# lisqzqng/Video-based-gait-analysis-for-dementia

Hardware: AMD Instinct MI355X
Metric: frames/sec (224x224, seq=16) (higher is better)
Workload: dtype f32

## Files before the change

include/grnet_hip.h:

```cpp
#ifndef GRNET_HIP_H
#define GRNET_HIP_H

#include <stddef.h>
#include <stdint.h>

#ifdef __cplusplus
extern "C" {
#endif

typedef struct grnet grnet_t;

#define GRNET_OK 0
#define GRNET_EINVAL (-22)
#define GRNET_ENOENT (-2)
#define GRNET_ENOMEM (-12)
#define GRNET_EHIP (-5)
#define GRNET_ESTATE (-1)

#define GRNET_DTYPE_F32 0
#define GRNET_DTYPE_I64 1

int grnet_create(grnet_t** out_handle, int device_id, int dtype, int max_frames);

#define GRNET_PRECISION_F32 0
// ... 7 lines not shown
int grnet_arena_fill(grnet_t* h, uint32_t pattern, void* stream);
int grnet_arena_assign(int n, const int64_t* sizes, int n_pairs, const int32_t* conflict_pairs, int64_t* offsets, int64_t* total);

int grnet_load_tensor(grnet_t* h, const char* state_dict_key, const void* host_ptr, const int64_t* shape, int ndim,
                      int dtype);

int grnet_load_smpl(grnet_t* h, const float* v_template, const float* shapedirs, const float* posedirs,
                    const float* J_regressor, const float* lbs_weights, const int32_t* parents,
                    const float* J_regressor_extra);

int grnet_finalize_weights(grnet_t* h);

typedef struct grnet_outputs {
    float* theta;
    float* verts;
    float* kp_2d;
    float* kp_3d;
    float* rotmat;
    float* point_local_feat;
    float* cam_shape_feats;
    float* pred_rot6d;
    float* features;
    float* part_attn;
    float* smpl_feats;
} grnet_outputs_t;

int grnet_forward(grnet_t* h, const float* frames_dev, int n_frames, const grnet_outputs_t* out, void* stream);

int grnet_gru_forward(grnet_t* h, const float* x_dev, const float* cparams_dev, int b, int T, float* y_dev,
                      float* phase_dev, float* xc_dev, void* stream);

int grnet_tsattn_forward(grnet_t* h, const float* x_dev, const float* xs_dev, int b, int n, float* y_dev, void* stream);

int grnet_tsattn_plan(grnet_t* h, int n, int32_t* plan);

int grnet_temporal_taps(grnet_t* h, float* buf_dev, size_t floats);

int grnet_temporal_tap_layout(grnet_t* h, char* buf, int buf_size);

#define GRNET_OPT_USE_GRAPH 1
#define GRNET_OPT_CONV_TILE 2
#define GRNET_OPT_MULTI_LANE 3
#define GRNET_OPT_WINOGRAD 7
#define GRNET_OPT_BF16_CHAIN 8
#define GRNET_OPT_GRU_MODE 9
#define GRNET_OPT_BF16_MIN_FRAMES 10
int grnet_set_option(grnet_t* h, int option, int value);

int grnet_tune(grnet_t* h, int n_frames, void* stream, int level );
int grnet_get_tuning(grnet_t* h, int n_frames, char* buf, int buf_size);
int grnet_set_tuning(grnet_t* h, int n_frames, const char* text);

int grnet_num_kernel_launches(grnet_t* h);
int grnet_num_conv_launches(grnet_t* h);
double grnet_conv_flops_per_frame(grnet_t* h);
double grnet_conv_executed_flops_per_frame(grnet_t* h);
double grnet_conv_executed_flops_per_frame_n(grnet_t* h, int n_frames);
int grnet_describe_conv(grnet_t* h, int pos, int32_t* info , char* name, int name_size);
double grnet_describe_conv_macs(grnet_t* h, int pos);
int grnet_conv_kernel_info(grnet_t* h, int pos, int n_frames, char* name, int name_size, double* executed_macs_per_frame);
int grnet_time_conv(grnet_t* h, int pos, int n_frames, int reps, void* stream, float* us_out);
int grnet_conv_launch_form(grnet_t* h, int pos, int n_frames, char* buf, int size, int* tuning_index);
int grnet_op_timeline(grnet_t* h, const float* frames_dev, int n_frames, void* stream, char* buf, int buf_size);
int grnet_time_convs(grnet_t* h, int n_frames, void* stream, float* ms_out);

int grnet_op_conv2d(grnet_t* h, const float* in_dev, int n, int cin, int hgt, int wid, const float* w_host,
                    const float* bias_host, int cout, int ks, int stride, int relu, const float* add_dev,
                    float* out_dev, int tile_hint, void* stream);
int grnet_op_conv2d_adds(grnet_t* h, const float* in_dev, int n, int cin, int hgt, int wid, const float* w_host, const float* bias_host, int cout, int ks,
                         int stride, int relu, int n_add, const float* const* adds_dev, const int* add_ctot, const int* add_coff, const int* add_shift,
                         float* out_dev, int tile_hint, void* stream);
int grnet_op_bilinear2x(grnet_t* h, const float* in_dev, int n, int c, int hgt, int wid, float* out_dev, void* stream);
int grnet_op_conv_chain(grnet_t* h, const float* in_dev, int n, int c, int wid, int nconv, const float* w_host, const float* bias_host,
                        float* out_dev, int reps, float* us_out, void* stream);

int grnet_smpl_forward(grnet_t* h, const float* betas_dev, const float* rotmat_dev, const float* cam_dev, int n, float* verts_dev,
                       float* kp3d_dev, float* kp2d_dev, void* stream);

#define GRNET_JOINT_REGRESSOR_MAX_ROWS 64
int grnet_set_joint_regressor(grnet_t* h, const float* J_host, int rows, const int32_t* select, int n_select);
int grnet_joint_regressor_rows(grnet_t* h);
int grnet_regress_joints(grnet_t* h, const float* verts_dev, int n, float* joints_dev, void* stream);

int grnet_head_forward(grnet_t* h, const float* point_local_feat_dev, const float* cam_shape_feats_dev, int n, const grnet_outputs_t* out,
                       void* stream);
typedef struct grnet_gait_outputs {
    float* pred_avg;
    float* pred_phase;
    float* pred_cparam;
    float* point_local_feat;
} grnet_gait_outputs_t;
int grnet_gait_correct(grnet_t* h, const float* point_local_feat_dev, const float* cam_shape_feats_dev, const float* cam_dev, int cam_ld,
                       const float* bbox_dev, const float* cimg_dev, int b, int T, const grnet_outputs_t* out,
                       const grnet_gait_outputs_t* gait, void* stream);

int grnet_op_rot6d_to_rotmat(grnet_t* h, const float* rot6d_dev, int m, float* rotmat_dev, void* stream);
int grnet_op_rotmat_to_aa(grnet_t* h, const float* rotmat_dev, int m, float* aa_dev, void* stream);
int grnet_op_aa_to_rotmat(grnet_t* h, const float* aa_dev, int m, float* rotmat_dev, void* stream);

int grnet_op_one_euro(grnet_t* h, const float* x_dev, int ld, int T, float min_cutoff, float beta, float d_cutoff, float* xhat_dev, void* stream);

#define GRNET_JOINTS_SPIN49   0
#define GRNET_JOINTS_SPIN2    1
#define GRNET_JOINTS_KINECTV2 2
int grnet_smooth_pose(grnet_t* h, const float* pose_dev, int pose_ld, const float* betas_dev, int T, float min_cutoff, float beta, int joints_kind,
                      float* pose_hat_dev, float* verts_dev, float* joints_dev, void* stream);
// ... 39 lines not shown
```

video-based-gait-analysis-for-dementia_amd/_lib.py:

```python
import ctypes as C
import os

_HERE = os.path.dirname(os.path.abspath(__file__))
LIB_PATH = os.environ.get("GRNET_LIB_PATH") or os.path.join(_HERE, "libgrnet_hip.so")

OK, EINVAL, ENOENT, ENOMEM, EHIP, ESTATE = 0, -22, -2, -12, -5, -1
DTYPE_F32, DTYPE_I64 = 0, 1
PRECISION_F32, PRECISION_BF16 = 0, 1
CREATE_COMPACT_ARENA = 1
JOINT_REGRESSOR_MAX_ROWS = 64
JOINTS_SPIN49, JOINTS_SPIN2, JOINTS_KINECTV2 = 0, 1, 2
RASTER_MAX_DIM, RASTER_SLOTS = 4096, 16
OPT_USE_GRAPH, OPT_CONV_TILE, OPT_MULTI_LANE, OPT_WINOGRAD, OPT_BF16_CHAIN, OPT_GRU_MODE, OPT_BF16_MIN_FRAMES = 1, 2, 3, 7, 8, 9, 10


class Outputs(C.Structure):
    _fields_ = [(n, C.c_void_p) for n in (
        "theta", "verts", "kp_2d", "kp_3d", "rotmat", "point_local_feat", "cam_shape_feats", "pred_rot6d",
        "features", "part_attn", "smpl_feats")]


class GaitOutputs(C.Structure):
    _fields_ = [(n, C.c_void_p) for n in ("pred_avg", "pred_phase", "pred_cparam", "point_local_feat")]


EXPORTS = {
    "grnet_create": (C.c_int, [C.POINTER(C.c_void_p), C.c_int, C.c_int, C.c_int]),
    "grnet_create_ex": (C.c_int, [C.POINTER(C.c_void_p), C.c_int, C.c_int, C.c_int, C.c_uint]),
    "grnet_arena_query": (C.c_int, [C.c_int, C.c_int, C.c_uint, C.POINTER(C.c_int64)]),
    "grnet_arena_layout": (C.c_int, [C.c_int, C.c_int, C.c_uint, C.c_char_p, C.c_int]),
    "grnet_arena_info": (C.c_int, [C.c_void_p, C.POINTER(C.c_int64)]),
    "grnet_arena_fill": (C.c_int, [C.c_void_p, C.c_uint32, C.c_void_p]),
    "grnet_arena_assign": (C.c_int, [C.c_int, C.POINTER(C.c_int64), C.c_int, C.POINTER(C.c_int32), C.POINTER(C.c_int64),
                                     C.POINTER(C.c_int64)]),
    "grnet_load_tensor": (C.c_int, [C.c_void_p, C.c_char_p, C.c_void_p, C.POINTER(C.c_int64), C.c_int, C.c_int]),
    "grnet_load_smpl": (C.c_int, [C.c_void_p] + [C.c_void_p] * 7),
    "grnet_finalize_weights": (C.c_int, [C.c_void_p]),
    "grnet_forward": (C.c_int, [C.c_void_p, C.c_void_p, C.c_int, C.POINTER(Outputs), C.c_void_p]),
    "grnet_gru_forward": (C.c_int, [C.c_void_p, C.c_void_p, C.c_void_p, C.c_int, C.c_int, C.c_void_p, C.c_void_p,
                                    C.c_void_p, C.c_void_p]),
    "grnet_tsattn_forward": (C.c_int, [C.c_void_p, C.c_void_p, C.c_void_p, C.c_int, C.c_int, C.c_void_p, C.c_void_p]),
    "grnet_tsattn_plan": (C.c_int, [C.c_void_p, C.c_int, C.POINTER(C.c_int32)]),
    "grnet_temporal_taps": (C.c_int, [C.c_void_p, C.c_void_p, C.c_size_t]),
    "grnet_temporal_tap_layout": (C.c_int, [C.c_void_p, C.c_char_p, C.c_int]),
    "grnet_set_option": (C.c_int, [C.c_void_p, C.c_int, C.c_int]),
    "grnet_tune": (C.c_int, [C.c_void_p, C.c_int, C.c_void_p, C.c_int]),
    "grnet_get_tuning": (C.c_int, [C.c_void_p, C.c_int, C.c_char_p, C.c_int]),
    "grnet_set_tuning": (C.c_int, [C.c_void_p, C.c_int, C.c_char_p]),
    "grnet_num_kernel_launches": (C.c_int, [C.c_void_p]),
    "grnet_num_conv_launches": (C.c_int, [C.c_void_p]),
    "grnet_conv_flops_per_frame": (C.c_double, [C.c_void_p]),
    "grnet_conv_executed_flops_per_frame": (C.c_double, [C.c_void_p]),
    "grnet_describe_conv": (C.c_int, [C.c_void_p, C.c_int, C.POINTER(C.c_int32), C.c_char_p, C.c_int]),
    "grnet_describe_conv_macs": (C.c_double, [C.c_void_p, C.c_int]),
    "grnet_conv_executed_flops_per_frame_n": (C.c_double, [C.c_void_p, C.c_int]),
    "grnet_conv_kernel_info": (C.c_int, [C.c_void_p, C.c_int, C.c_int, C.c_char_p, C.c_int, C.POINTER(C.c_double)]),
    "grnet_time_conv": (C.c_int, [C.c_void_p, C.c_int, C.c_int, C.c_int, C.c_void_p, C.POINTER(C.c_float)]),
    "grnet_conv_launch_form": (C.c_int, [C.c_void_p, C.c_int, C.c_int, C.c_char_p, C.c_int, C.POINTER(C.c_int)]),
    "grnet_op_timeline": (C.c_int, [C.c_void_p, C.c_void_p, C.c_int, C.c_void_p, C.c_char_p, C.c_int]),
    "grnet_time_convs": (C.c_int, [C.c_void_p, C.c_int, C.c_void_p, C.POINTER(C.c_float)]),
    "grnet_op_conv2d": (C.c_int, [C.c_void_p, C.c_void_p, C.c_int, C.c_int, C.c_int, C.c_int, C.c_void_p, C.c_void_p,
                                  C.c_int, C.c_int, C.c_int, C.c_int, C.c_void_p, C.c_void_p, C.c_int, C.c_void_p]),
    "grnet_op_conv2d_adds": (C.c_int, [C.c_void_p, C.c_void_p, C.c_int, C.c_int, C.c_int, C.c_int, C.c_void_p, C.c_void_p, C.c_int, C.c_int,
                                       C.c_int, C.c_int, C.c_int, C.POINTER(C.c_void_p), C.POINTER(C.c_int), C.POINTER(C.c_int),
                                       C.POINTER(C.c_int), C.c_void_p, C.c_int, C.c_void_p]),
    "grnet_op_conv_chain": (C.c_int, [C.c_void_p, C.c_void_p, C.c_int, C.c_int, C.c_int, C.c_int, C.c_void_p, C.c_void_p, C.c_void_p, C.c_int,
                                      C.POINTER(C.c_float), C.c_void_p]),
    "grnet_op_bilinear2x": (C.c_int, [C.c_void_p, C.c_void_p, C.c_int, C.c_int, C.c_int, C.c_int, C.c_void_p, C.c_void_p]),
    "grnet_smpl_forward": (C.c_int, [C.c_void_p, C.c_void_p, C.c_void_p, C.c_void_p, C.c_int, C.c_void_p, C.c_void_p, C.c_void_p,
                                     C.c_void_p]),
    "grnet_crop_normalise": (C.c_int, [C.c_void_p, C.c_void_p, C.c_int, C.c_int, C.c_int, C.c_int, C.c_void_p, C.c_float, C.c_int,
                                       C.c_void_p, C.c_void_p]),
    "grnet_crop_normalise_cv": (C.c_int, [C.c_void_p, C.c_void_p, C.c_int, C.c_int, C.c_int, C.c_int, C.c_void_p, C.c_int, C.c_void_p,
                                          C.c_void_p]),
    "grnet_crop_normalise_cv_maps": (C.c_int, [C.c_void_p, C.c_void_p, C.c_int, C.c_int, C.c_int, C.c_int, C.c_void_p, C.c_int, C.c_void_p,
                                          C.c_void_p]),
    "grnet_head_forward": (C.c_int, [C.c_void_p, C.c_void_p, C.c_void_p, C.c_int, C.POINTER(Outputs), C.c_void_p]),
    "grnet_gait_correct": (C.c_int, [C.c_void_p, C.c_void_p, C.c_void_p, C.c_void_p, C.c_int, C.c_void_p, C.c_void_p, C.c_int, C.c_int,
                                     C.POINTER(Outputs), C.POINTER(GaitOutputs), C.c_void_p]),
    "grnet_set_joint_regressor": (C.c_int, [C.c_void_p, C.c_void_p, C.c_int, C.POINTER(C.c_int32), C.c_int]),
    "grnet_joint_regressor_rows": (C.c_int, [C.c_void_p]),
    "grnet_regress_joints": (C.c_int, [C.c_void_p, C.c_void_p, C.c_int, C.c_void_p, C.c_void_p]),
    "grnet_op_rot6d_to_rotmat": (C.c_int, [C.c_void_p, C.c_void_p, C.c_int, C.c_void_p, C.c_void_p]),
    "grnet_op_rotmat_to_aa": (C.c_int, [C.c_void_p, C.c_void_p, C.c_int, C.c_void_p, C.c_void_p]),
    "grnet_op_aa_to_rotmat": (C.c_int, [C.c_void_p, C.c_void_p, C.c_int, C.c_void_p, C.c_void_p]),
    "grnet_op_one_euro": (C.c_int, [C.c_void_p, C.c_void_p, C.c_int, C.c_int, C.c_float, C.c_float, C.c_float, C.c_void_p, C.c_void_p]),
    "grnet_smooth_pose": (C.c_int, [C.c_void_p, C.c_void_p, C.c_int, C.c_void_p, C.c_int, C.c_float, C.c_float, C.c_int, C.c_void_p, C.c_void_p,
                                    C.c_void_p, C.c_void_p]),
    "grnet_load_faces": (C.c_int, [C.c_void_p, C.c_void_p, C.c_int]),
    "grnet_render_meshes": (C.c_int, [C.c_void_p, C.c_void_p, C.c_int, C.c_void_p, C.c_void_p, C.c_void_p, C.c_void_p, C.c_void_p, C.c_int, C.c_int,
                                      C.c_int, C.c_void_p]),
    "grnet_op_raster_setup": (C.c_int, [C.c_void_p, C.c_void_p, C.c_int, C.c_void_p, C.c_int, C.c_void_p, C.c_void_p, C.c_int, C.c_int, C.c_void_p,
                                        C.c_void_p, C.c_void_p, C.c_void_p]),
    "grnet_op_raster": (C.c_int, [C.c_void_p, C.c_void_p, C.c_void_p, C.c_int, C.c_void_p, C.c_int, C.c_int, C.c_int, C.c_void_p, C.c_void_p]),
    "grnet_debug_tensor": (C.c_int, [C.c_void_p, C.c_char_p, C.c_int, C.c_void_p, C.POINTER(C.c_int64), C.c_void_p]),
    "grnet_comm_probe": (C.c_int, []),
    "grnet_comm_unique_id": (C.c_int, [C.c_void_p, C.c_int]),
    "grnet_comm_create": (C.c_int, [C.POINTER(C.c_void_p), C.c_void_p, C.c_int, C.c_int, C.c_int]),
    "grnet_comm_adopt": (C.c_int, [C.POINTER(C.c_void_p), C.c_void_p, C.c_int, C.c_int]),
    "grnet_allgather": (C.c_int, [C.c_void_p, C.c_void_p, C.c_void_p, C.c_size_t, C.c_void_p]),
    "grnet_comm_info": (C.c_int, [C.c_void_p, C.POINTER(C.c_int), C.POINTER(C.c_int)]),
    "grnet_comm_destroy": (None, [C.c_void_p]),
# ... 44 lines not shown
```

video-based-gait-analysis-for-dementia_amd/csrc/grnet.cpp:

```cpp
#include "grnet_impl.h"

static bool copy_text(const std::string& s, char* buf, int size) {
    if ((int)s.size() + 1 > size) return false;
    memcpy(buf, s.c_str(), s.size() + 1);
    return true;
}

grnet::~grnet() {
    for (auto& g : graphs) (void)hipGraphExecDestroy(g.second.exec);
    if (capture_stream) (void)hipStreamDestroy(capture_stream);
    for (int l = 1; l < kLanes; ++l) {
        if (side[l]) (void)hipStreamDestroy(side[l]);
        if (ev_join[l]) (void)hipEventDestroy(ev_join[l]);
    }
    if (ev_fork) (void)hipEventDestroy(ev_fork);
    for (hipEvent_t e : op_events_flat) if (e) (void)hipEventDestroy(e);
    for (void* p : dev_allocs) (void)hipFree(p);
    jreg_clear();
    faces_clear();
    if (raster_ws) (void)hipFree(raster_ws);
    if (temporal_ws) (void)hipFree(temporal_ws);
    if (gru_fault) (void)hipHostFree(gru_fault);
    if (arena) (void)hipFree(arena);
}
// ... 273 lines not shown
        h->gru_mode = value;
        return 0;
    }
    if (option == GRNET_OPT_BF16_MIN_FRAMES) {
        if (value < 0) return h->fail(GRNET_EINVAL, "the smallest call of the bf16 kernel groups is >= 1 frame (0: each group's own default)");
        h->bf16_min_frames = value;
        h->drop_graphs();
        return 0;
    }
    if (option == GRNET_OPT_MULTI_LANE) {
        h->multi_lane = value != 0;
        h->drop_graphs();
        return 0;
    }
    return h->fail(GRNET_EINVAL, "unknown option");
}

int grnet_tune(grnet_t* h, int n_frames, void* stream, int level) {
    if (!h) return GRNET_EINVAL;
    DeviceGuard guard(h->device);
    return h->tune(n_frames, static_cast<hipStream_t>(stream), level);
}

int grnet_get_tuning(grnet_t* h, int n_frames, char* buf, int buf_size) {
    if (!h || !buf || buf_size < 16) return GRNET_EINVAL;
    auto m = h->tuned_mode.find(n_frames);
    if (m == h->tuned_mode.end()) return h->fail(GRNET_ESTATE, "no tuning for this n_frames");
    std::string out = "mode " + std::to_string(m->second) + "\n";
    for (size_t i = 0; i < h->convs.size(); ++i) {
        auto it = h->convs[i].tuned.find(n_frames);
        out += std::to_string(i) + " " + std::to_string(it == h->convs[i].tuned.end() ? 0 : it->second) + "\n";
    }
    if (!copy_text(out, buf, buf_size)) return h->fail(GRNET_EINVAL, "buffer too small");
    return (int)out.size();
}

int grnet_set_tuning(grnet_t* h, int n_frames, const char* text) {
    if (!h || !text) return GRNET_EINVAL;
    int mode = 0, consumed = 0;
    if (sscanf(text, "mode %d\n%n", &mode, &consumed) != 1) return h->fail(GRNET_EINVAL, "bad tuning text");
    const char* p = text + consumed;
    int idx, hint, used;
    while (sscanf(p, "%d %d\n%n", &idx, &hint, &used) == 2) {
        if (idx < 0 || idx >= (int)h->convs.size()) return h->fail(GRNET_EINVAL, "tuning text does not match this plan");
        h->convs[idx].tuned[n_frames] = hint;
        p += used;
    }
    h->tuned_mode[n_frames] = mode;
    h->drop_graphs();
    return 0;
}

int grnet_num_kernel_launches(grnet_t* h) { return h ? h->launches_last : GRNET_EINVAL; }

int grnet_num_conv_launches(grnet_t* h) { return h ? (int)(h->convs.size() + h->fuse_ups.size()) : GRNET_EINVAL; }

double grnet_conv_flops_per_frame(grnet_t* h) {
    if (!h) return 0;
    double m = 0;
    for (auto& L : h->convs) m += L.macs_per_frame;
    for (auto& fp : h->fuse_ups) m += fp.macs_per_frame;
    return 2.0 * m;
}

double grnet_conv_executed_flops_per_frame_n(grnet_t* h, int n_frames) {
    if (!h) return 0;
    double m = 0;
    for (auto& L : h->convs) m += L.macs_per_frame * h->executed_ratio(L, n_frames);
    for (auto& fp : h->fuse_ups) m += fp.macs_per_frame;
    return 2.0 * m;
}

double grnet_conv_executed_flops_per_frame(grnet_t* h) { return h ? grnet_conv_executed_flops_per_frame_n(h, h->last_n) : 0; }

int grnet_describe_conv(grnet_t* h, int pos, int32_t* info, char* name, int name_size) {
    if (!h || !info || !h->finalized || pos < 0) return GRNET_EINVAL;
    const Op* found = h->nth_conv_op(pos);
    if (!found) return GRNET_EINVAL;
    const Op& op = *found;
    if (op.kind == Op::FUSEUP) {
        const FuseUpPlan& fp = h->fuse_ups[op.conv_idx];
        int cout = 0;
        int64_t rd = 0;
        for (int i = 0; i < fp.nb - 1; ++i) cout += kBranchCh[i];
        for (int j = 0; j < fp.nb; ++j) rd += (int64_t)kBranchCh[j] * fp.xs[j].h * fp.xs[j].w;
        const int32_t v[12] = {0, cout, 1, 1, fp.xs[0].h, fp.xs[0].w, fp.xs[0].h, fp.xs[0].w, fp.nb, 1, op.lane, (int32_t)rd};
        memcpy(info, v, sizeof(v));
        if (name && name_size > 0) snprintf(name, name_size, "%sfuse_layers(up)", fp.prefix.c_str());
        return 0;
    }
    const ConvLayer& L = h->convs[op.conv_idx];
    int64_t add_elems = 0;
    for (const AddRef& r : L.adds) add_elems += (int64_t)L.cout * (L.out.h >> r.shift) * (L.out.w >> r.shift);
    const int32_t v[12] = {L.in.c + L.in2.c, L.cout, L.ks, L.stride, L.in.h, L.in.w, L.out.h, L.out.w, (int32_t)L.adds.size(), L.relu,
                           op.lane, (int32_t)add_elems};
    memcpy(info, v, sizeof(v));
    if (name && name_size > 0) snprintf(name, name_size, "%s", L.segs.empty() ? "" : L.segs[0].wkey.c_str());
    return 0;
}

double grnet_describe_conv_macs(grnet_t* h, int pos) {
    if (!h || pos < 0) return -1.0;
    const Op* op = h->nth_conv_op(pos);
    if (!op) return -1.0;
    return op->kind == Op::FUSEUP ? h->fuse_ups[op->conv_idx].macs_per_frame : h->convs[op->conv_idx].macs_per_frame;
}
// ... 245 lines not shown
```

video-based-gait-analysis-for-dementia_amd/csrc/grnet_impl.h:

```cpp
#pragma once
#include "../../include/grnet_hip.h"

#include <hip/hip_runtime.h>

#include <cmath>
#include <cstdio>
#include <cstdlib>
#include <algorithm>
#include <cstring>
#include <map>
#include <memory>
#include <string>
#include <tuple>
#include <unordered_map>
#include <vector>

#include "kernels.h"

namespace grnet_detail {
using namespace grk;

inline uint16_t f32_to_bf16(float f) {
    uint32_t u;
    memcpy(&u, &f, 4);
// ... 128 lines not shown
    int conv_tile_hint = 0;
    int wino_mode = 1;
    static constexpr int kChainModeAll = 1023;
    int chain_mode = (getenv("GRNET_BF16_CHAIN") ? atoi(getenv("GRNET_BF16_CHAIN")) : kChainModeAll) & kChainModeAll;
    int bf16_min_frames = 0;
    int gru_mode = 3;
    unsigned* gru_fault = nullptr;
    unsigned* gru_fault_dev = nullptr;

    std::vector<ConvLayer> convs;
    std::vector<Op> ops;
    std::vector<size_t> buffer_floats;
    std::vector<FuseUpPlan> fuse_ups;
    std::vector<ChainPlan> chains;
    std::vector<RollPlan> rolls;
    struct SumPlan { View out; std::vector<AddRef> adds; };
    std::vector<SumPlan> sum_views;
    std::vector<std::pair<std::string, View>> named;
    std::vector<int> end_reads;
    View v_input, v_cat, v_heat, v_smpl_feats, v_csmap;
    View v_in8;
    bool bf16_stem = false;
    int cur_lane = 0;
    bool solo_region = false;

    static constexpr int64_t kArenaHead = 64, kArenaTail = 64, kArenaAlign = 64;
    ArenaPlan arena_plan;
    float* arena = nullptr;
    size_t arena_floats = 0;
    std::vector<void*> dev_allocs;
    float* zeros = nullptr;
    float *d_plf = nullptr, *d_csf = nullptr, *d_stats = nullptr, *d_rot6d = nullptr, *d_shape = nullptr, *d_cam = nullptr;
    float *d_rotmat = nullptr, *d_theta = nullptr, *d_A = nullptr, *d_verts = nullptr, *d_kp3d = nullptr, *d_kp2d = nullptr;

    std::unordered_map<std::string, HostTensor> tensors;
    TailWeights tailw{};
    SmplTables smpl{};
    GruWeights gruw{};
    TsAttnWeights tsw{};
    FeatCorrWeights fcw{};
    std::vector<float> J_regressor_host;
    float *jreg_pack = nullptr, *jreg_ws = nullptr;
    int jreg_rows = 0;
    float* smooth_ws = nullptr;
    RasterMesh rmesh{};
    void* rmesh_block = nullptr;
    void* raster_ws = nullptr;

    std::vector<Op> ops_flat;
    std::vector<hipEvent_t> op_events_flat;
    hipStream_t side[kLanes] = {};
    hipEvent_t ev_fork = nullptr, ev_join[kLanes] = {};
    int lanes_used = 1;
    int launches_last = 0;
    int last_n = 16;
    std::map<int, int> tuned_mode;
    struct GraphKey {
        int n; const void* in; grnet_outputs_t o;
        bool operator<(const GraphKey& r) const {
            if (n != r.n) return n < r.n;
            if (in != r.in) return in < r.in;
            return std::memcmp(&o, &r.o, sizeof(o)) < 0;
        }
    };
    struct GraphEntry { hipGraphExec_t exec; unsigned long long last_use; };
    std::map<GraphKey, GraphEntry> graphs;
    unsigned long long graph_clock = 0;
    std::vector<GraphKey> seen_once;
    hipStream_t capture_stream = nullptr;
    std::vector<hipEvent_t>* tl_start = nullptr;
    std::vector<hipEvent_t>* tl_end = nullptr;

    float* temporal_ws = nullptr;
    size_t temporal_ws_floats = 0;
    TapSink tap_sink;
    bool taps_armed = false;

    int fail(int code, const std::string& msg) {
        err = msg;
        return code;
    }
    static View slice(View v, int coff, int c) {
        v.coff += coff;
        v.c = c;
        return v;
    }
    void name_view(const std::string& n, const View& v) { named.emplace_back(n, v); }
    float* base(const View& v, const float* frames = nullptr) const {
        if (v.slot >= 0) return arena + arena_plan.off[v.slot];
        return v.slot == View::kFrames ? const_cast<float*>(frames) : nullptr;
    }
    template <class P>
    void bind(const View& v, P*& p, int& ctot, int& coff, const float* frames = nullptr) const { p = base(v, frames); ctot = v.ctot; coff = v.coff; }
    const void* bf16_at(const View& v) const { return reinterpret_cast<const uint16_t*>(base(v)) + v.coff; }
    bool pair_active(int n) const { return dtype == 1 && (chain_mode & 64) && !conv_tile_hint && (long)n * 56 * 56 >= 256L * 112 * 2; }

    View new_buffer(int c, int h, int w);
    View add_conv(View in, std::vector<ConvSeg> segs, int ks, int stride, bool relu, std::vector<AddRef> adds = {}, const View* out_override = nullptr);
    View conv_bn(View in, const std::string& wkey, const std::string& bn, int cout, int ks, int stride, bool relu, std::vector<AddRef> adds = {},
                 const View* out_override = nullptr);
    View add_bilinear(View in);
    std::vector<View> hr_module(std::vector<View> xs, const std::string& p, const View* out0);
    std::vector<View> hr_fuse_grouped(const std::vector<View>& xs, const std::string& p, const View* out0, const std::vector<int>& branch_tail);
    std::vector<View> hr_fuse_separate(std::vector<View> xs, const std::string& p, const View* out0, bool up0 = false, const std::vector<int>& branch_tail = {});
    void add_roll(int kind, int n_convs);
    void build_plan();
// ... 72 lines not shown
```

video-based-gait-analysis-for-dementia_amd/csrc/grnet_plan.cpp:

```cpp
#include "grnet_impl.h"

View grnet::new_buffer(int c, int h, int w) {
    const int ct = dtype == 1 ? (c + 7) / 8 * 8 : c;
    View v;
    v.slot = (int)buffer_floats.size();
    v.ctot = ct; v.coff = 0; v.c = c; v.h = h; v.w = w;
    buffer_floats.push_back((size_t)ct * h * w);
    return v;
}

View grnet::add_conv(View in, std::vector<ConvSeg> segs, int ks, int stride, bool relu, std::vector<AddRef> adds,
                     const View* out_override) {
    ConvLayer L;
    L.in = in;
    int cout = 0;
    for (auto& s : segs) cout += s.cout;
    const int pad = ks / 2;
    const int ho = (in.h + 2 * pad - ks) / stride + 1, wo = (in.w + 2 * pad - ks) / stride + 1;
    L.out = out_override ? *out_override : new_buffer(cout, ho, wo);
    L.segs = std::move(segs);
    L.cout = cout; L.ks = ks; L.stride = stride; L.relu = relu;
    L.adds = std::move(adds);
    L.cin_w = (dtype == 1 && in.c == 8 && in.ctot == 8) ? 3 : in.c;
    L.macs_per_frame = (double)ho * wo * cout * L.cin_w * ks * ks;
    L.lane_hint = cur_lane;
    L.solo = solo_region;
    convs.push_back(L);
    Op op;
    op.kind = Op::CONV;
    op.conv_idx = (int)convs.size() - 1;
    op.lane = cur_lane;
    ops.push_back(op);
    return convs.back().out;
}
View grnet::conv_bn(View in, const std::string& wkey, const std::string& bn, int cout, int ks, int stride, bool relu,
                    std::vector<AddRef> adds, const View* out_override) {
    return add_conv(in, {ConvSeg{wkey, bn, "", cout}}, ks, stride, relu, std::move(adds), out_override);
}

View grnet::add_bilinear(View in) {
    View out = new_buffer(in.c, in.h * 2, in.w * 2);
    Op op;
    op.kind = Op::BILINEAR;
    op.bin = in; op.bout = out;
    op.lane = cur_lane;
    ops.push_back(op);
    return out;
}

std::vector<View> grnet::hr_module(std::vector<View> xs, const std::string& p, const View* out0) {
    const int nb = (int)xs.size();
    std::vector<int> branch_tail(nb, -1);
    cur_lane = 0;
// ... 665 lines not shown
    static const int n_lanes = std::min(kLanes, std::max(1, GRNET_AB(LANES, 4)));
    order.reserve(m);
    for (int step = 0; step < m; ++step) {
        int best = -1, best_lane = 0;
        double best_start = 0;
        for (int i = 0; i < m; ++i) {
            if (done[i] || pending[i]) continue;
            double ready = 0;
            int from = -1;
            for (int d : deps[i])
                if (finish[d] >= ready) { ready = finish[d]; from = d; }
            const bool pinned = list[i].kind == Op::POOL || list[i].kind == Op::TAIL || list[i].kind == Op::SMPL;
            int lane = 0;
            double start = std::max(ready, lane_free[0]);
            if (!pinned && list[i].follow >= 0) {
                lane = lane_of[list[i].follow];
                start = std::max(ready, lane_free[lane]);
            } else if (!pinned) {
                const int pref = from >= 0 ? lane_of[from] : 0;
                lane = pref;
                start = std::max(ready, lane_free[pref]);
                for (int l = 0; l < n_lanes; ++l) {
                    const double st = std::max(ready, lane_free[l]);
                    if (st + hop_us < start) { start = st; lane = l; }
                }
            }
            if (best < 0 || start < best_start - 1e-9 || (start < best_start + 1e-9 && blevel[i] > blevel[best])) {
                best = i; best_lane = lane; best_start = start;
            }
        }
        done[best] = 1;
        lane_of[best] = best_lane;
        finish[best] = best_start + est[best];
        lane_free[best_lane] = finish[best];
        for (int u : users[best]) --pending[u];
        order.push_back(best);
    }
    std::vector<Op> out;
    out.reserve(m);
    for (int i : order) {
        Op op = list[i];
        op.lane = lane_of[i];
        op.waits.clear();
        op.record = false;
        out.push_back(std::move(op));
    }
    if (getenv("GRNET_TRACE")) fprintf(stderr, "[grnet] lane schedule: %d ops, estimated makespan %.0f us (sum of estimates %.0f us)\n", m,
                                       *std::max_element(lane_free, lane_free + kLanes), [&] { double t = 0; for (double e : est) t += e; return t; }());
    list.swap(out);
}

void grnet::analyze_dependencies(std::vector<Op>& ops, std::vector<hipEvent_t>& op_events) {
    const std::vector<std::vector<int>> producers = raw_producers(ops);
    for (int i = 0; i < (int)ops.size(); ++i)
        for (int w : producers[i])
            if (ops[w].lane != ops[i].lane) {
                ops[i].waits.push_back(w);
                ops[w].record = true;
            }
    op_events.assign(ops.size(), nullptr);
    if (getenv("GRNET_TRACE")) {
        size_t waits = 0, records = 0;
        for (const Op& op : ops) { waits += op.waits.size(); records += op.record; }
        fprintf(stderr, "[grnet] dependencies: %zu ops, %zu cross-lane waits, %zu recorded events\n", ops.size(), waits, records);
    }
}
```

video-based-gait-analysis-for-dementia_amd/csrc/grnet_run.cpp:

```cpp
#include "grnet_impl.h"

namespace grk { thread_local GraphRecorder* g_recorder = nullptr; }

int grnet::allocate() {
    if (plan_arena(compact, arena_plan)) return fail(GRNET_ESTATE, "the activation arena could not be planned: a launch group or the assignment violates the sharing rule");
    const size_t total = (size_t)arena_plan.total;
    arena_floats = total;
    void* q = nullptr;
    if (hipMalloc(&q, total * sizeof(float)) != hipSuccess)
        return fail(GRNET_ENOMEM, std::string("hipMalloc of the ") + (compact ? "compact " : "") + "activation arena (" + std::to_string(total * 4 >> 20) + " MiB) failed");
    arena = static_cast<float*>(q);
    if (hipMemset(arena, 0, 64 * sizeof(float)) != hipSuccess) return fail(GRNET_EHIP, "hipMemset failed");
    zeros = arena;
    if (hipEventCreateWithFlags(&ev_fork, hipEventDisableTiming) != hipSuccess) return fail(GRNET_EHIP, "hipEventCreate failed");
    if (int rc = install_schedule(max_frames)) return rc;
    if (hipStreamCreateWithFlags(&capture_stream, hipStreamNonBlocking) != hipSuccess) return fail(GRNET_EHIP, "hipStreamCreate failed");
    const size_t n = max_frames;
    int rc;
    if ((rc = dev_alloc(&d_plf, n * 128 * 24))) return rc;
    if ((rc = dev_alloc(&d_csf, n * 64 * 24))) return rc;
    if ((rc = dev_alloc(&d_stats, softmax_pool_ws_floats((int)n)))) return rc;
    if ((rc = dev_alloc(&d_rot6d, n * 144))) return rc;
    if ((rc = dev_alloc(&d_shape, n * 10))) return rc;
    if ((rc = dev_alloc(&d_cam, n * 3))) return rc;
// ... 240 lines not shown
    }
    return 0;
}
int grnet::launch_fuse_up_op(const FuseUpPlan& fp, int n, hipStream_t s) {
    FuseUpArgs a{};
    a.N = n; a.nb = fp.nb; a.only = fp.only;
    for (int i = 0; i < fp.nb - 1; ++i) {
        if (fp.only >= 0 && fp.only != i) continue;
        FuseUpOut& fo = a.o[i];
        bind(fp.outs[i], fo.out, fo.out_ctot, fo.out_coff);
        bind(fp.xs[i], fo.base, fo.base_ctot, fo.base_coff);
        fo.bias = fp.b_dev[i];
        fo.relu = 1;
        fo.n_extra = (int)fp.extra[i].size();
        for (int k = 0; k < fo.n_extra; ++k) bind(fp.extra[i][k], fo.extra[k], fo.extra_ctot[k], fo.extra_coff[k]);
        for (int j = i + 1; j < fp.nb; ++j) {
            FuseUpSrc& src = fo.src[j - i - 1];
            bind(fp.xs[j], src.x, src.ctot, src.coff);
            src.w = fp.w_dev[i][j - i - 1];
        }
    }
    HIP_TRY(dtype == 1 ? launch_hr_fuse_up_bf16(a, s) : launch_hr_fuse_up(a, s));
    return 0;
}

grnet::HeadOutputs grnet::head_outputs(const grnet_outputs_t& o) const {
    return {o.pred_rot6d ? o.pred_rot6d : d_rot6d, o.rotmat ? o.rotmat : d_rotmat, o.theta ? o.theta : d_theta,
            o.verts ? o.verts : d_verts,           o.kp_3d ? o.kp_3d : d_kp3d,     o.kp_2d ? o.kp_2d : d_kp2d};
}

int grnet::enqueue(const float* frames, int n, const grnet_outputs_t& o, hipStream_t s, bool convs_only) {
    int launches = 0;
    last_n = n;
    float* plf = o.point_local_feat ? o.point_local_feat : d_plf;
    float* csf = o.cam_shape_feats ? o.cam_shape_feats : d_csf;
    const auto [rot6d, rotmat, theta, verts, kp3d, kp2d] = head_outputs(o);
    const std::vector<Op>& ops = ops_flat;
    const std::vector<hipEvent_t>& op_events = op_events_flat;
    GraphRecorder* rec = g_recorder;
    const bool lanes = multi_lane && !rec;
    std::vector<hipGraphNode_t> lane_last(kLanes, nullptr), op_node(rec ? ops.size() : 0, nullptr);
    hipStream_t lane_stream[kLanes];
    for (int l = 0; l < kLanes; ++l) lane_stream[l] = s;
    if (lanes) {
        HIP_TRY(hipEventRecord(ev_fork, s));
        for (int l = 1; l < lanes_used; ++l) {
            lane_stream[l] = side[l];
            HIP_TRY(hipStreamWaitEvent(side[l], ev_fork, 0));
        }
    }
    hipStream_t caller = s;
    for (size_t oi = 0; oi < ops.size(); ++oi) {
        const Op& op = ops[oi];
        if (convs_only && op.kind != Op::CONV && op.kind != Op::FUSEUP) continue;
        s = lane_stream[op.lane];
        const int lane = multi_lane ? op.lane : 0;
        if (lanes)
            for (int w : op.waits) HIP_TRY(hipStreamWaitEvent(s, op_events[w], 0));
        if (tl_start && !rec) HIP_TRY(hipEventRecord((*tl_start)[oi], s));
        if (rec) {
            rec->deps.clear();
            rec->n_chain = lane_last[lane] ? 1 : 0;
            if (lane_last[lane]) rec->deps.push_back(lane_last[lane]);
            if (multi_lane)
                for (int w : op.waits)
                    if (op_node[w] && std::find(rec->deps.begin(), rec->deps.end(), op_node[w]) == rec->deps.end()) rec->deps.push_back(op_node[w]);
        }
        static const char* abl_skip = GRNET_AB_STR(ABL_SKIP);
        if (abl_skip && (op.kind == Op::CONV || op.kind == Op::FUSEUP)) {
            const std::string lbl = op_label(op);
            bool skip = false;
            for (const char* q = abl_skip; *q;) {
                const char* e = strchr(q, ',');
                const std::string pat = e ? std::string(q, e) : std::string(q);
                if (!pat.empty() && lbl.find(pat) != std::string::npos) skip = true;
                q = e ? e + 1 : q + strlen(q);
            }
            if (skip) {
                if (tl_end && !rec) HIP_TRY(hipEventRecord((*tl_end)[oi], s));
                if (lanes && op.record) HIP_TRY(hipEventRecord(op_events[oi], s));
                continue;
            }
        }
        switch (op.kind) {
            case Op::CONVERT:
                HIP_TRY(launch_nchw_f32_to_nhwc_bf16(frames, base(v_in8), n, 3, 224, 224, 8, s));
                ++launches;
                break;
            case Op::CONV: {
                int nl = 1;
                if (int rc = launch_conv_op(convs[op.conv_idx], frames, n, s, &nl)) return rc;
                launches += nl;
                break;
            }
            case Op::SUM: {
                const auto& sv = sum_views[op.conv_idx];
                SumArgs a = op.sum;
                a.N = n;
                bind(sv.out, a.out, a.out_ctot, a.out_coff);
                for (int k = 0; k < a.n_add; ++k) {
                    bind(sv.adds[k].v, a.add[k], a.add_ctot[k], a.add_coff[k]);
                    a.add_shift[k] = sv.adds[k].shift;
                }
                if (dtype == 1) HIP_TRY(launch_fuse_sum_bf16(a, s));
                else HIP_TRY(launch_fuse_sum(a, s));
                ++launches;
                break;
            }
            case Op::FUSEUP:
                if (int rc = launch_fuse_up_op(fuse_ups[op.conv_idx], n, s)) return rc;
                ++launches;
                break;
            case Op::BILINEAR:
                if (dtype == 1) HIP_TRY(launch_bilinear2x_bf16(base(op.bin), base(op.bout), n, op.bin.c, op.bin.h, op.bin.w, s));
                else HIP_TRY(launch_bilinear2x(base(op.bin), base(op.bout), n, op.bin.c, op.bin.h, op.bin.w, s));
                ++launches;
                break;
            case Op::POOL:
                if (dtype == 1)
                    HIP_TRY(launch_softmax_pool_bf16(base(v_heat), v_heat.ctot, bf16_at(v_smpl_feats), 128, v_smpl_feats.ctot, bf16_at(v_csmap), 64,
                                                     v_csmap.ctot, d_stats, n, 56 * 56, s));
                else
                    HIP_TRY(launch_softmax_pool(base(v_heat), 25, base(v_smpl_feats), 128, base(v_csmap), 64, plf, csf, d_stats, n, 56 * 56, s));
                ++launches;
                break;
            case Op::TAIL:
                HIP_TRY(launch_head_tail(d_stats, true, plf, csf, tailw, rot6d, d_shape, d_cam, rotmat, theta, n, s));
                ++launches;
                break;
            case Op::SMPL:
                HIP_TRY(launch_smpl(d_shape, rotmat, d_cam, smpl, d_A, verts, kp3d, kp2d, n, s));
                launches += 4;
                break;
        }
        if (tl_end && !rec) HIP_TRY(hipEventRecord((*tl_end)[oi], s));
        if (lanes && op.record) HIP_TRY(hipEventRecord(op_events[oi], s));
        if (rec && !rec->deps.empty()) lane_last[lane] = op_node[oi] = rec->deps[0];
    }
    s = caller;
    if (lanes)
        for (int l = 1; l < lanes_used; ++l) {
            HIP_TRY(hipEventRecord(ev_join[l], side[l]));
            HIP_TRY(hipStreamWaitEvent(s, ev_join[l], 0));
        }
    if (!convs_only) {
        auto copy_out = [&](float* dst, const float* src, size_t bytes) -> int {
            if (!dst) return 0;
            if (!rec) { HIP_TRY(hipMemcpyAsync(dst, src, bytes, hipMemcpyDeviceToDevice, s)); return 0; }
            std::vector<hipGraphNode_t> deps;
            for (hipGraphNode_t nd : lane_last) if (nd) deps.push_back(nd);
            hipGraphNode_t node = nullptr;
            HIP_TRY(hipGraphAddMemcpyNode1D(&node, rec->graph, deps.data(), deps.size(), dst, src, bytes, hipMemcpyDeviceToDevice));
            return 0;
        };
        int rc;
        if (dtype == 1) {
            auto conv_out = [&](float* dst, const View& v) -> int {
                if (!dst) return 0;
                if (rec) {
                    rec->deps.clear();
                    for (hipGraphNode_t nd : lane_last) if (nd) rec->deps.push_back(nd);
                }
                HIP_TRY(launch_nhwc_bf16_to_nchw_f32(base(v), dst, n, v.c, v.h, v.w, v.ctot, v.coff, s));
                return 0;
            };
            if ((rc = conv_out(o.features, v_cat))) return rc;
            if ((rc = conv_out(o.part_attn, v_heat))) return rc;
            if ((rc = conv_out(o.smpl_feats, v_smpl_feats))) return rc;
        } else {
        if ((rc = copy_out(o.features, base(v_cat), (size_t)n * 480 * 3136 * 4))) return rc;
        if ((rc = copy_out(o.part_attn, base(v_heat), (size_t)n * 25 * 3136 * 4))) return rc;
        if ((rc = copy_out(o.smpl_feats, base(v_smpl_feats), (size_t)n * 128 * 3136 * 4))) return rc;
        }
        launches_last = launches;
    }
    return 0;
}

int grnet::head_from_feats(const float* plf, const float* csf, int n, const grnet_outputs_t& o, hipStream_t s) {
    const auto [rot6d, rotmat, theta, verts, kp3d, kp2d] = head_outputs(o);
    HIP_TRY(launch_head_tail_from_feats(plf, csf, tailw, rot6d, d_shape, d_cam, rotmat, theta, n, s));
    HIP_TRY(launch_smpl(d_shape, rotmat, d_cam, smpl, d_A, verts, kp3d, kp2d, n, s));
    if (o.point_local_feat && o.point_local_feat != plf) HIP_TRY(hipMemcpyAsync(o.point_local_feat, plf, (size_t)n * 3072 * 4, hipMemcpyDeviceToDevice, s));
    if (o.cam_shape_feats && o.cam_shape_feats != csf) HIP_TRY(hipMemcpyAsync(o.cam_shape_feats, csf, (size_t)n * 1536 * 4, hipMemcpyDeviceToDevice, s));
    return 0;
}

int grnet::gait_correct(const float* plf, const float* csf, const float* cam, int cam_ld, const float* bbox, const float* cimg, int b, int T,
                        const grnet_outputs_t& o, const grnet_gait_outputs_t& g, hipStream_t s) {
    if (int rc = gru_fault_check()) return rc;
    const size_t M = (size_t)b * T;
    const bool taps = taps_armed;
    if (taps) {
        size_t need = 0;
// ... 268 lines not shown
```

video-based-gait-analysis-for-dementia_amd/grnet.py:

```python
import ctypes as C
import logging
from collections import namedtuple

import numpy as np
import torch

from . import _lib, netspec

logger = logging.getLogger(__name__)
_IncompatibleKeys = namedtuple("_IncompatibleKeys", ["missing_keys", "unexpected_keys"])

SMPL_PREFIX = "regressor.smpl.smpl."
_SMPL_KEYS = ("v_template", "shapedirs", "posedirs", "J_regressor", "lbs_weights", "parents", "J_regressor_extra")
_TOLERATED_SMPL_KEYS = ("vertex_joint_selector.extra_joints_idxs", "betas", "global_orient",
                        "body_pose", "transl")


def _np32(t):
    if torch.is_tensor(t):
        t = t.detach().cpu().numpy()
    return np.ascontiguousarray(np.asarray(t), dtype=np.float32)


def reference_selection(rows):
# ... 301 lines not shown
    def gait_correct(self, point_local_feat, cam_shape_feats, theta_or_cam, bbox, cimg, b, t):
        self.finalize()
        dev, m = self.device, b * t
        f = lambda x, *shape: x.to(dev, torch.float32).reshape(*shape).contiguous()
        plf, csf = f(point_local_feat, m, 128, 24), f(cam_shape_feats, m, 64, 24)
        cam = f(theta_or_cam, m, -1)
        bb, ci = f(bbox, m, 4), f(cimg, m, 2)
        new = lambda *s: torch.empty(s, dtype=torch.float32, device=dev)
        out = {"theta": new(m, 85), "verts": new(m, 6890, 3), "kp_2d": new(m, 29, 2), "kp_3d": new(m, 29, 3), "rotmat": new(m, 24, 3, 3)}
        gait = {"pred_avg": new(b, 3), "pred_phase": new(b, t, 4), "pred_cparam": new(m, 3), "point_local_feat": new(m, 128, 24)}
        o, g = _lib.Outputs(), _lib.GaitOutputs()
        for k, v in out.items():
            setattr(o, k, v.data_ptr())
        for k, v in gait.items():
            setattr(g, k, v.data_ptr())
        stream = C.c_void_p(torch.cuda.current_stream(dev).cuda_stream)
        rc = self._lib.grnet_gait_correct(self._h, plf.data_ptr(), csf.data_ptr(), cam.data_ptr(), cam.shape[1], bb.data_ptr(), ci.data_ptr(),
                                          b, t, C.byref(o), C.byref(g), stream)
        _lib.check(self._lib, self._h, rc, "grnet_gait_correct")
        out.update(gait)
        return out

    def tune(self, n_frames, level=1, cache=None):
        self.finalize()
        import os
        if cache and os.path.isfile(cache):
            with open(cache) as f:
                rc = self._lib.grnet_set_tuning(self._h, int(n_frames), f.read().encode())
            if rc == 0:
                return self
        stream = C.c_void_p(torch.cuda.current_stream(self.device).cuda_stream)
        _lib.check(self._lib, self._h, self._lib.grnet_tune(self._h, int(n_frames), stream, int(level)), "grnet_tune")
        if cache:
            buf = C.create_string_buffer(1 << 16)
            if self._lib.grnet_get_tuning(self._h, int(n_frames), buf, len(buf)) > 0:
                os.makedirs(os.path.dirname(os.path.abspath(cache)), exist_ok=True)
                with open(cache, "w") as f:
                    f.write(buf.value.decode())
        return self

    def tuned_mode(self, n_frames):
        buf = C.create_string_buffer(1 << 16)
        if self._lib.grnet_get_tuning(self._h, int(n_frames), buf, len(buf)) <= 0:
            return None
        mode = int(buf.value.decode().split("\n", 1)[0].split()[1])
        return {"measured_table": bool(mode & 1), "eager": bool(mode & 4)}

    def num_kernel_launches(self):
        return self._lib.grnet_num_kernel_launches(self._h)

    def num_conv_launches(self):
        return self._lib.grnet_num_conv_launches(self._h)

    def conv_flops_per_frame(self):
        return self._lib.grnet_conv_flops_per_frame(self._h)

    def conv_executed_flops_per_frame(self, n_frames=None):
        self.finalize()
        if n_frames is None:
            return self._lib.grnet_conv_executed_flops_per_frame(self._h)
        return self._lib.grnet_conv_executed_flops_per_frame_n(self._h, int(n_frames))

    def kernel_table(self, n_frames, reps=20):
        self.finalize()
        stream = C.c_void_p(torch.cuda.current_stream(self.device).cuda_stream)
        convs = self.describe_convs()
        timed, rows = {}, {}
        for pos, c in enumerate(convs):
            name, ex = C.create_string_buffer(96), C.c_double()
            _lib.check(self._lib, self._h, self._lib.grnet_conv_kernel_info(self._h, pos, int(n_frames), name, 96, C.byref(ex)), "grnet_conv_kernel_info")
            key = (name.value, c["cin"], c["cout"], c["ks"], c["stride"], c["hin"], c["n_add"], c["macs"])
            if key not in timed:
                us = C.c_float()
                _lib.check(self._lib, self._h, self._lib.grnet_time_conv(self._h, pos, int(n_frames), int(reps), stream, C.byref(us)), "grnet_time_conv")
                timed[key] = us.value
            member = name.value.endswith(b"+")
            row = name.value.decode().rstrip("+")
            r = rows.setdefault(row, {"name": row, "launches": 0, "total_us": 0.0, "gflop": 0.0, "executed_gflop": 0.0})
            r["launches"] += 0 if member else 1
            r["total_us"] += timed[key]
            r["gflop"] += 2.0 * c["macs"] * n_frames / 1e9
            r["executed_gflop"] += 2.0 * ex.value * n_frames / 1e9
        out = sorted(rows.values(), key=lambda r: -r["total_us"])
        for r in out:
            r["avg_us"] = r["total_us"] / r["launches"]
        return out

    def conv_kernels(self, n_frames):
        self.finalize()
        out = []
        for pos, c in enumerate(self.describe_convs()):
            name = C.create_string_buffer(96)
            _lib.check(self._lib, self._h, self._lib.grnet_conv_kernel_info(self._h, pos, int(n_frames), name, 96, None), "grnet_conv_kernel_info")
            out.append((c["name"], name.value.decode()))
        return out

    def conv_launch_forms(self, n_frames):
        self.finalize()
        out = []
        for pos, c in enumerate(self.describe_convs()):
            out.append((c["name"],) + self.conv_launch_form(pos, n_frames))
        return out

    def conv_launch_form(self, pos, n_frames):
        buf, idx = C.create_string_buffer(256), C.c_int(-1)
        _lib.check(self._lib, self._h, self._lib.grnet_conv_launch_form(self._h, int(pos), int(n_frames), buf, len(buf), C.byref(idx)), "grnet_conv_launch_form")
# ... 402 lines not shown
```

Before: 4519.

## Prune redundant cross-lane event waits and final lane joins using vector clocks

Replaces the all-pairs cross-lane wait generation with a vector-clock transitive reduction. A wait is dropped when an earlier wait on the same lane, or one carried by another producer, already implies it, and lanes whose last op is already observed by the main lane skip the final join. This cuts hipStreamWaitEvent/hipEventRecord calls and graph edges in the multi-lane schedule. It also adds a plan-count query API, and in convs-only mode non-conv ops still honour waits and records. The risk is a missed dependency if the clock reasoning is wrong, for example the join check reads clock[l], which is lane 0's view of lane l.

After: 4581 (median of 6 runs). 1.01x the previous value.

```diff
diff --git a/include/grnet_hip.h b/include/grnet_hip.h
--- a/include/grnet_hip.h
+++ b/include/grnet_hip.h
@@ -83,6 +83,8 @@
 int grnet_set_tuning(grnet_t* h, int n_frames, const char* text);
 
 int grnet_num_kernel_launches(grnet_t* h);
+enum { GRNET_PLAN_OPS = 0, GRNET_PLAN_WAITS_ALL, GRNET_PLAN_RECORDS_ALL, GRNET_PLAN_WAITS, GRNET_PLAN_RECORDS, GRNET_PLAN_LANES_ALL, GRNET_PLAN_LANES_JOINED, GRNET_PLAN_COUNTS };
+int grnet_plan_counts(grnet_t* h, int64_t* counts );
 int grnet_num_conv_launches(grnet_t* h);
 double grnet_conv_flops_per_frame(grnet_t* h);
 double grnet_conv_executed_flops_per_frame(grnet_t* h);
diff --git a/video-based-gait-analysis-for-dementia_amd/_lib.py b/video-based-gait-analysis-for-dementia_amd/_lib.py
--- a/video-based-gait-analysis-for-dementia_amd/_lib.py
+++ b/video-based-gait-analysis-for-dementia_amd/_lib.py
@@ -10,6 +10,7 @@
 CREATE_COMPACT_ARENA = 1
 JOINT_REGRESSOR_MAX_ROWS = 64
 JOINTS_SPIN49, JOINTS_SPIN2, JOINTS_KINECTV2 = 0, 1, 2
+PLAN_COUNTS = ("ops", "waits_all", "records_all", "waits", "records", "lanes_all", "lanes_joined")
 RASTER_MAX_DIM, RASTER_SLOTS = 4096, 16
 OPT_USE_GRAPH, OPT_CONV_TILE, OPT_MULTI_LANE, OPT_WINOGRAD, OPT_BF16_CHAIN, OPT_GRU_MODE, OPT_BF16_MIN_FRAMES = 1, 2, 3, 7, 8, 9, 10
 
@@ -48,6 +49,7 @@
     "grnet_get_tuning": (C.c_int, [C.c_void_p, C.c_int, C.c_char_p, C.c_int]),
     "grnet_set_tuning": (C.c_int, [C.c_void_p, C.c_int, C.c_char_p]),
     "grnet_num_kernel_launches": (C.c_int, [C.c_void_p]),
+    "grnet_plan_counts": (C.c_int, [C.c_void_p, C.POINTER(C.c_int64)]),
     "grnet_num_conv_launches": (C.c_int, [C.c_void_p]),
     "grnet_conv_flops_per_frame": (C.c_double, [C.c_void_p]),
     "grnet_conv_executed_flops_per_frame": (C.c_double, [C.c_void_p]),
diff --git a/video-based-gait-analysis-for-dementia_amd/csrc/grnet.cpp b/video-based-gait-analysis-for-dementia_amd/csrc/grnet.cpp
--- a/video-based-gait-analysis-for-dementia_amd/csrc/grnet.cpp
+++ b/video-based-gait-analysis-for-dementia_amd/csrc/grnet.cpp
@@ -349,6 +349,12 @@
 }
 
 int grnet_num_kernel_launches(grnet_t* h) { return h ? h->launches_last : GRNET_EINVAL; }
+
+int grnet_plan_counts(grnet_t* h, int64_t* counts) {
+    if (!h || !counts) return GRNET_EINVAL;
+    std::copy(h->handoff_counts, h->handoff_counts + GRNET_PLAN_COUNTS, counts);
+    return 0;
+}
 
 int grnet_num_conv_launches(grnet_t* h) { return h ? (int)(h->convs.size() + h->fuse_ups.size()) : GRNET_EINVAL; }
 
diff --git a/video-based-gait-analysis-for-dementia_amd/csrc/grnet_impl.h b/video-based-gait-analysis-for-dementia_amd/csrc/grnet_impl.h
--- a/video-based-gait-analysis-for-dementia_amd/csrc/grnet_impl.h
+++ b/video-based-gait-analysis-for-dementia_amd/csrc/grnet_impl.h
@@ -204,6 +204,8 @@
     hipStream_t side[kLanes] = {};
     hipEvent_t ev_fork = nullptr, ev_join[kLanes] = {};
     int lanes_used = 1;
+    bool join_lane[kLanes] = {};
+    int64_t handoff_counts[GRNET_PLAN_COUNTS] = {};
     int launches_last = 0;
     int last_n = 16;
     std::map<int, int> tuned_mode;
diff --git a/video-based-gait-analysis-for-dementia_amd/csrc/grnet_plan.cpp b/video-based-gait-analysis-for-dementia_amd/csrc/grnet_plan.cpp
--- a/video-based-gait-analysis-for-dementia_amd/csrc/grnet_plan.cpp
+++ b/video-based-gait-analysis-for-dementia_amd/csrc/grnet_plan.cpp
@@ -1,4 +1,5 @@
 #include "grnet_impl.h"
+#include "lane_deps.h"
 
 View grnet::new_buffer(int c, int h, int w) {
     const int ct = dtype == 1 ? (c + 7) / 8 * 8 : c;
@@ -770,16 +771,31 @@
 
 void grnet::analyze_dependencies(std::vector<Op>& ops, std::vector<hipEvent_t>& op_events) {
     const std::vector<std::vector<int>> producers = raw_producers(ops);
-    for (int i = 0; i < (int)ops.size(); ++i)
-        for (int w : producers[i])
-            if (ops[w].lane != ops[i].lane) {
-                ops[i].waits.push_back(w);
-                ops[w].record = true;
-            }
+    std::vector<int> lane_of(ops.size());
+    for (size_t i = 0; i < ops.size(); ++i) lane_of[i] = ops[i].lane;
+    static const int reduce_waits = GRNET_AB(WAIT_REDUCE, 1);
+    const lane_deps::Handoffs all = lane_deps::all_cross_lane_waits(lane_of, producers);
+    const lane_deps::Handoffs kept = reduce_waits ? lane_deps::reduce_cross_lane_waits(lane_of, producers) : all;
+    for (size_t i = 0; i < ops.size(); ++i) {
+        ops[i].waits = kept.waits[i];
+        ops[i].record = kept.record[i] != 0;
+    }
+    std::fill(join_lane, join_lane + kLanes, false);
+    int joins_all = 0, joins_kept = 0;
+    for (size_t l = 1; l < kept.join.size() && l < (size_t)kLanes; ++l) {
+        join_lane[l] = kept.join[l] != 0;
+        joins_all += all.join[l];
+        joins_kept += kept.join[l];
+    }
+    handoff_counts[GRNET_PLAN_OPS] = (int64_t)ops.size();
+    handoff_counts[GRNET_PLAN_WAITS_ALL] = (int64_t)all.n_waits;
+    handoff_counts[GRNET_PLAN_RECORDS_ALL] = (int64_t)all.n_records;
+    handoff_counts[GRNET_PLAN_WAITS] = (int64_t)kept.n_waits;
+    handoff_counts[GRNET_PLAN_RECORDS] = (int64_t)kept.n_records;
+    handoff_counts[GRNET_PLAN_LANES_ALL] = joins_all;
+    handoff_counts[GRNET_PLAN_LANES_JOINED] = joins_kept;
     op_events.assign(ops.size(), nullptr);
-    if (getenv("GRNET_TRACE")) {
-        size_t waits = 0, records = 0;
-        for (const Op& op : ops) { waits += op.waits.size(); records += op.record; }
-        fprintf(stderr, "[grnet] dependencies: %zu ops, %zu cross-lane waits, %zu recorded events\n", ops.size(), waits, records);
-    }
-}
+    if (getenv("GRNET_TRACE"))
+        fprintf(stderr, "[grnet] dependencies: %zu ops, cross-lane waits %zu -> %zu, recorded events %zu -> %zu, joined lanes %d -> %d\n", ops.size(), all.n_waits,
+                kept.n_waits, all.n_records, kept.n_records, joins_all, joins_kept);
+}
diff --git a/video-based-gait-analysis-for-dementia_amd/csrc/grnet_run.cpp b/video-based-gait-analysis-for-dementia_amd/csrc/grnet_run.cpp
--- a/video-based-gait-analysis-for-dementia_amd/csrc/grnet_run.cpp
+++ b/video-based-gait-analysis-for-dementia_amd/csrc/grnet_run.cpp
@@ -316,11 +316,14 @@
     hipStream_t caller = s;
     for (size_t oi = 0; oi < ops.size(); ++oi) {
         const Op& op = ops[oi];
-        if (convs_only && op.kind != Op::CONV && op.kind != Op::FUSEUP) continue;
         s = lane_stream[op.lane];
         const int lane = multi_lane ? op.lane : 0;
         if (lanes)
             for (int w : op.waits) HIP_TRY(hipStreamWaitEvent(s, op_events[w], 0));
+        if (convs_only && op.kind != Op::CONV && op.kind != Op::FUSEUP) {
+            if (lanes && op.record) HIP_TRY(hipEventRecord(op_events[oi], s));
+            continue;
+        }
         if (tl_start && !rec) HIP_TRY(hipEventRecord((*tl_start)[oi], s));
         if (rec) {
             rec->deps.clear();
@@ -404,6 +407,7 @@
     s = caller;
     if (lanes)
         for (int l = 1; l < lanes_used; ++l) {
+            if (!join_lane[l]) continue;
             HIP_TRY(hipEventRecord(ev_join[l], side[l]));
             HIP_TRY(hipStreamWaitEvent(s, ev_join[l], 0));
         }
diff --git a/video-based-gait-analysis-for-dementia_amd/csrc/lane_deps.h b/video-based-gait-analysis-for-dementia_amd/csrc/lane_deps.h
--- /dev/null
+++ b/video-based-gait-analysis-for-dementia_amd/csrc/lane_deps.h
@@ -0,0 +1,81 @@
+#pragma once
+#include <algorithm>
+#include <vector>
+
+namespace lane_deps {
+
+struct Handoffs {
+    std::vector<std::vector<int>> waits;
+    std::vector<char> record;
+    std::vector<char> join;
+    size_t n_waits = 0, n_records = 0;
+};
+
+inline void count(Handoffs& h) {
+    h.n_waits = h.n_records = 0;
+    for (const auto& w : h.waits) h.n_waits += w.size();
+    for (char r : h.record) h.n_records += r != 0;
+}
+
+inline int lane_count(const std::vector<int>& lane_of) {
+    int lanes = 1;
+    for (int l : lane_of) lanes = std::max(lanes, l + 1);
+    return lanes;
+}
+
+inline Handoffs all_cross_lane_waits(const std::vector<int>& lane_of, const std::vector<std::vector<int>>& producers) {
+    const int m = (int)lane_of.size();
+    Handoffs h;
+    h.waits.assign(m, {});
+    h.record.assign(m, 0);
+    h.join.assign(lane_count(lane_of), 0);
+    for (int i = 0; i < m; ++i) {
+        if (lane_of[i] > 0) h.join[lane_of[i]] = 1;
+        for (int w : producers[i])
+            if (lane_of[w] != lane_of[i]) {
+                h.waits[i].push_back(w);
+                h.record[w] = 1;
+            }
+    }
+    count(h);
+    return h;
+}
+
+inline Handoffs reduce_cross_lane_waits(const std::vector<int>& lane_of, const std::vector<std::vector<int>>& producers) {
+    const int m = (int)lane_of.size(), lanes = lane_count(lane_of);
+    Handoffs h;
+    h.waits.assign(m, {});
+    h.record.assign(m, 0);
+    h.join.assign(lanes, 0);
+    std::vector<int> clock((size_t)lanes * lanes, -1);
+    std::vector<int> snap((size_t)m * lanes, -1);
+    std::vector<int> last(lanes, -1), cand;
+    for (int i = 0; i < m; ++i) {
+        const int a = lane_of[i];
+        int* mine = &clock[(size_t)a * lanes];
+        cand.clear();
+        for (int w : producers[i])
+            if (lane_of[w] != a) cand.push_back(w);
+        for (int w : cand) {
+            const int b = lane_of[w];
+            bool implied = mine[b] >= w;
+            for (size_t k = 0; k < cand.size() && !implied; ++k)
+                implied = cand[k] != w && snap[(size_t)cand[k] * lanes + b] >= w;
+            if (!implied) {
+                h.waits[i].push_back(w);
+                h.record[w] = 1;
+            }
+        }
+        for (int w : h.waits[i])
+            for (int c = 0; c < lanes; ++c)
+                if (c != a) mine[c] = std::max(mine[c], snap[(size_t)w * lanes + c]);
+        std::copy(mine, mine + lanes, &snap[(size_t)i * lanes]);
+        snap[(size_t)i * lanes + a] = i;
+        last[a] = i;
+    }
+    for (int l = 1; l < lanes; ++l) h.join[l] = last[l] >= 0 && clock[l] < last[l];
+    count(h);
+    return h;
+}
+
+}
diff --git a/video-based-gait-analysis-for-dementia_amd/grnet.py b/video-based-gait-analysis-for-dementia_amd/grnet.py
--- a/video-based-gait-analysis-for-dementia_amd/grnet.py
+++ b/video-based-gait-analysis-for-dementia_amd/grnet.py
@@ -377,6 +377,11 @@
     def num_conv_launches(self):
         return self._lib.grnet_num_conv_launches(self._h)
 
+    def plan_counts(self):
+        c = (C.c_int64 * len(_lib.PLAN_COUNTS))()
+        _lib.check(self._lib, self._h, self._lib.grnet_plan_counts(self._h, c), "grnet_plan_counts")
+        return dict(zip(_lib.PLAN_COUNTS, (int(v) for v in c)))
+
     def conv_flops_per_frame(self):
         return self._lib.grnet_conv_flops_per_frame(self._h)
 
```
